# 0x002A/MuCHSALSA

Hardware: AMD Instinct MI355X
Metric: overlap-pairs/s (higher is better)
Workload: dtype int32+f64; 1 GPU; 100k synthetic Nanopore x10 kb, 500k unitig anchors, 10x coverage (BASELINE.json configs[2]); rows=5059558, reads=100000, anchors=499992, edges=981460, edgematches_rank0=25532466, orders_rank0=1029308, parallelism=one job on one GPU, edges_proven_clean_rank0=5372

## Files before the change

muchsalsa_amd/csrc/msgpu_device.h:

```cpp
#ifndef MSGPU_DEVICE_H
#define MSGPU_DEVICE_H

#include <hip/hip_runtime.h>
#include <stdint.h>

#include "msgpu.h"
#include "msgpu_internal.h"

namespace msgpu {

__device__ __forceinline__ IRow load_irow(const IRow *p) {
  const uint4 *q = reinterpret_cast<const uint4 *>(p);
  uint4        a = q[0], b = q[1];
  IRow         r;
  r.n_lo  = static_cast<int>(a.x);
  r.n_hi  = static_cast<int>(a.y);
  r.i_lo  = static_cast<int>(a.z);
  r.i_hi  = static_cast<int>(a.w);
  r.score = b.x;
  r.line  = b.y;
  r.other = b.z;
  r.pf    = b.w;
  return r;
}
__device__ __forceinline__ void store_irow(IRow *p, const IRow &r) {
  uint4 *q = reinterpret_cast<uint4 *>(p);
  q[0]     = make_uint4(static_cast<uint32_t>(r.n_lo), static_cast<uint32_t>(r.n_hi), static_cast<uint32_t>(r.i_lo),
                        static_cast<uint32_t>(r.i_hi));
  q[1]     = make_uint4(r.score, r.line, r.other, r.pf);
}

__device__ __forceinline__ IRow make_irow(const msgpu_row &row, uint32_t other, uint32_t rank) {
  IRow out;
  out.n_lo  = row.n_lo;
  out.n_hi  = row.n_hi;
  out.i_lo  = row.i_lo;
  out.i_hi  = row.i_hi;
  out.score = row.score;
  out.line  = row.line;
  out.other = other;
  out.pf    = ((row.flags & MSGPU_ROW_DIR) ? PF_DIR : 0u) | ((row.flags & MSGPU_ROW_PRIMARY) ? PF_PRIM : 0u) |
           (rank & PF_POS_MASK);
  return out;
}

__device__ __forceinline__ int rl_i32(int v, int lane) { return __builtin_amdgcn_readlane(v, lane); }
__device__ __forceinline__ uint32_t rl_u32(uint32_t v, int lane) {
  return static_cast<uint32_t>(__builtin_amdgcn_readlane(static_cast<int>(v), lane));
}
__device__ __forceinline__ uint64_t rl_u64(uint64_t v, int lane) {
  uint32_t lo = rl_u32(static_cast<uint32_t>(v), lane), hi = rl_u32(static_cast<uint32_t>(v >> 32), lane);
  return (static_cast<uint64_t>(hi) << 32) | lo;
}
__device__ __forceinline__ double rl_f64(double v, int lane) {
  return __longlong_as_double(static_cast<long long>(rl_u64(static_cast<uint64_t>(__double_as_longlong(v)), lane)));
}

__device__ __forceinline__ void publish_to_host(const HostPublish &p, int lane, uint64_t v) {
  if (!p.seq) return;
  if (lane < SC_COUNT) p.host[lane] = v;
  __threadfence_system();
  if (lane == 0) __hip_atomic_store(&p.host[SC_COUNT], p.seq, __ATOMIC_RELEASE, __HIP_MEMORY_SCOPE_SYSTEM);
}

__device__ __forceinline__ double std_max(double a, double b) { return (a < b) ? b : a; }
__device__ __forceinline__ double std_min(double a, double b) { return (b < a) ? b : a; }

__device__ __forceinline__ uint32_t wave_incl_scan(uint32_t v) {
  v += static_cast<uint32_t>(__builtin_amdgcn_update_dpp(0, static_cast<int>(v), 0x111, 0xf, 0xf, false));
  v += static_cast<uint32_t>(__builtin_amdgcn_update_dpp(0, static_cast<int>(v), 0x112, 0xf, 0xf, false));
  v += static_cast<uint32_t>(__builtin_amdgcn_update_dpp(0, static_cast<int>(v), 0x114, 0xf, 0xf, false));
  v += static_cast<uint32_t>(__builtin_amdgcn_update_dpp(0, static_cast<int>(v), 0x118, 0xf, 0xf, false));
  v += static_cast<uint32_t>(__builtin_amdgcn_update_dpp(0, static_cast<int>(v), 0x142, 0xa, 0xf, false));
  v += static_cast<uint32_t>(__builtin_amdgcn_update_dpp(0, static_cast<int>(v), 0x143, 0xc, 0xf, false));
  return v;
}

__device__ __forceinline__ uint64_t wave_incl_scan64(uint32_t v) {
  uint64_t inc = v;
  const int lane = threadIdx.x & 63;
#pragma unroll
  for (int d = 1; d < 64; d <<= 1) {
    const uint64_t t = __shfl_up(inc, d);
    if (lane >= d) inc += t;
  }
  return inc;
}
__device__ __forceinline__ uint32_t wave_sum(uint32_t v) {
  return static_cast<uint32_t>(__builtin_amdgcn_readlane(static_cast<int>(wave_incl_scan(v)), 63));
}

template <int NT> __device__ __forceinline__ uint32_t block_excl_scan(uint32_t v, uint32_t *s_wave , uint32_t *total) {
  const int      lane = threadIdx.x & 63, wave = threadIdx.x >> 6;
  const uint32_t inc  = wave_incl_scan(v);
  if (lane == 63) s_wave[wave] = inc;
  __syncthreads();
  uint32_t base = 0, tot = 0;
#pragma unroll
  for (int w = 0; w < NT / 64; ++w) {
    const uint32_t x = s_wave[w];
    base += w < wave ? x : 0u;
    tot += x;
  }
  *total = tot;
  __syncthreads();
  return base + inc - v;
}
__device__ __forceinline__ uint32_t block_excl_scan_256(uint32_t v, uint32_t *s_wave , uint32_t *total) {
  const int lane = threadIdx.x & 63, wave = threadIdx.x >> 6;
  uint32_t  inc  = v;
#pragma unroll
  for (int d = 1; d < 64; d <<= 1) {
    uint32_t t = __shfl_up(inc, d);
    if (lane >= d) inc += t;
  }
  if (lane == 63) s_wave[wave] = inc;
  __syncthreads();
  uint32_t w0 = s_wave[0], w1 = s_wave[1], w2 = s_wave[2], w3 = s_wave[3];
  uint32_t base = (wave > 0 ? w0 : 0) + (wave > 1 ? w1 : 0) + (wave > 2 ? w2 : 0);
  *total        = w0 + w1 + w2 + w3;
  __syncthreads();
  return base + inc - v;
}

__device__ __forceinline__ void note_first_row(int lane, unsigned long long key, uint32_t r, const msgpu_row *rows,
                                               int32_t *read_len, uint32_t *read_first) {
  for (int d = 32; d > 0; d >>= 1) {
    const unsigned long long o =
        (static_cast<unsigned long long>(static_cast<uint32_t>(__shfl_xor(static_cast<int>(key >> 32), d))) << 32) |
        static_cast<uint32_t>(__shfl_xor(static_cast<int>(key), d));
    key = o < key ? o : key;
  }
  if (lane == 0) {
    read_first[r] = static_cast<uint32_t>(key >> 32);
    read_len[r]   = rows[static_cast<uint32_t>(key)].read_len;
  }
}

__device__ __forceinline__ bool key_less(int alo, int ahi, uint32_t aan, int blo, int bhi, uint32_t ban) {
  return alo < blo || (alo == blo && (ahi < bhi || (ahi == bhi && aan < ban)));
}

}

#endif
```

muchsalsa_amd/csrc/msgpu_kernels.hip:

```cpp
#include <hip/hip_runtime.h>
#include <stdint.h>
#include <stdlib.h>

#include <type_traits>
#include <utility>

#include "msgpu.h"
#include "msgpu_internal.h"
#include "msgpu_device.h"

namespace msgpu {


constexpr int SCAN_ITEMS = 8;
uint32_t      scan_blocks(uint64_t n);

template <class T> __global__ __launch_bounds__(256) void k_scan_reduce(const uint32_t *in, uint64_t n, T *block_sums) {
  __shared__ T s[4];
  uint64_t     base = static_cast<uint64_t>(blockIdx.x) * 256 * SCAN_ITEMS;
  T            sum  = 0;
  for (int i = 0; i < SCAN_ITEMS; ++i) {
    uint64_t idx = base + static_cast<uint64_t>(i) * 256 + threadIdx.x;
    if (idx < n) sum += in[idx];
  }
// ... 1290 lines not shown
}
void launch_emit_edges(hipStream_t st, const EmitArgs &a, bool reduce) {
  if (reduce && a.n_chunks)
    hipLaunchKernelGGL(k_cand_reduce, dim3(a.n_chunks), dim3(1024), 0, st, a.n_edge, a.n_cand, a.cand_off, a.edge_scr_start, a.V,
                       const_cast<unsigned long long *>(a.chunk_sums), const_cast<uint32_t *>(a.hist));
  hipLaunchKernelGGL(k_emit_edges, dim3(a.n_chunks ? a.n_chunks : 1), dim3(1024), 0, st, a);
}


__device__ __forceinline__ void chunk_add(unsigned long long *chunk_sums, uint64_t e, bool clean, uint32_t n_orders, uint32_t n_ids, bool banded = false) {
  static_assert(COMPACT_CHUNK < (1u << 16), "two 16-bit edge counts in the low half of a chunk sum");
  unsigned long long *c = chunk_sums + 2 * (e / COMPACT_CHUNK);
  __hip_atomic_fetch_add(c, (clean ? 1ull : 0ull) | (banded ? 1ull << 16 : 0ull) | (static_cast<unsigned long long>(n_orders) << 32), __ATOMIC_RELAXED, __HIP_MEMORY_SCOPE_AGENT);
  __hip_atomic_fetch_add(c + 1, static_cast<unsigned long long>(n_ids), __ATOMIC_RELAXED, __HIP_MEMORY_SCOPE_AGENT);
}
__device__ __forceinline__ void band_fallback_add(unsigned long long *chunk_sums, uint64_t n_edges) {
  __hip_atomic_fetch_add(chunk_sums + 2 * (n_edges / COMPACT_CHUNK + 1), 1ull, __ATOMIC_RELAXED, __HIP_MEMORY_SCOPE_AGENT);
}

struct PathRec {
  uint64_t mask;
  uint64_t score;
  uint32_t primary;
  uint32_t pad;
};

struct __attribute__((aligned(16))) ChainElem {
  double clo1, chi1;
  double clo2, chi2;
  int    rlo1, rhi1, rlo2, rhi2;
};

struct NanoMasks {
  unsigned long long pos, neg, ovl, abort_;
};
template <bool WF, int SORTED >
__device__ __forceinline__ NanoMasks nano_check(double k_clo, double k_chi, double l_clo, double l_chi, int k_rlo,
                                                int k_rhi, int l_rlo, int l_rhi, double &d) {
  typedef unsigned long long M;
  const bool lt_lo_b = k_clo < l_clo;
  const M    lt_lo = __ballot(lt_lo_b), lt_hi = __ballot(k_chi < l_chi);
  const M    gt_lo = __ballot(k_clo > l_clo), gt_hi = __ballot(k_chi > l_chi);
  NanoMasks  f;
  const double x = k_chi - l_clo;
  const double y = l_chi - k_clo;
  double       t = lt_lo_b ? x : y;
  if (WF) {
    f.ovl = __ballot(t >= 0.0);
    d     = fabs(t) + 1;
  } else {
    f.ovl = __ballot(k_clo <= l_chi) & __ballot(l_clo <= k_chi);
    t     = __builtin_amdgcn_inverse_ballot_w64(f.ovl) ? t : -t;
    d = t + 1;
  }
  if (WF) {
    f.pos = lt_lo & lt_hi;
    f.neg = gt_lo & gt_hi;
  } else {
    f.pos = lt_lo & (lt_hi | ~f.ovl);
    f.neg = (f.ovl & gt_lo & gt_hi) | ~(f.ovl | lt_lo);
  }
  if (SORTED == 1) {
    const M rovl = __ballot(l_rlo <= k_rhi);
    const M u2   = __ballot(k_rlo < l_rlo) & __ballot(k_rhi < l_rhi);
    f.abort_     = rovl & (f.neg | (f.pos & ~u2));
  } else if (SORTED == 2) {
    const M rovl = __ballot(k_rlo <= l_rhi);
    const M um2  = __ballot(k_rlo > l_rlo) & __ballot(k_rhi > l_rhi);
    f.abort_     = rovl & (f.pos | (f.neg & ~um2));
  } else {
    const M rovl = __ballot(k_rlo <= l_rhi) & __ballot(l_rlo <= k_rhi);
    const M u2   = __ballot(k_rlo < l_rlo) & __ballot(k_rhi < l_rhi);
    const M um2  = __ballot(k_rlo > l_rlo) & __ballot(k_rhi > l_rhi);
    f.abort_     = rovl & ((f.neg & ~um2) | (f.pos & ~u2));
  }
  return f;
}

__device__ __forceinline__ int paths_of_direction(unsigned long long act, bool direction, int lane, double pop,
                                                  uint64_t pm, bool em_prim, uint32_t j1, uint32_t q2, uint32_t n1,
                                                  uint32_t n2, double alt_frac, PathRec *paths) {
  if (act == 0) return 0;
  const bool mine = (act >> lane) & 1ull;
  double best = mine ? pop : -1.0;
#pragma unroll
  for (int d = 32; d > 0; d >>= 1) best = __builtin_fmax(best, __shfl_xor(best, d));
  double maxv;
  int    maxi;
  if (best > 0.0) {
    maxv = best;
    maxi = __builtin_ctzll(__ballot(mine && pop == best));
  } else {
    maxv = 0.0;
    maxi = __builtin_ctzll(act);
  }
  maxi = __builtin_amdgcn_readfirstlane(maxi);
  const unsigned long long prim_lanes = __ballot(mine && em_prim);
  int                      np         = 0;
  const uint64_t           m          = rl_u64(pm, maxi);
  bool                     hp         = (m & prim_lanes) != 0;
  hp |= __popcll(m) > 2;
  if (lane == 0) {
    paths[0].mask    = m;
    paths[0].score   = static_cast<uint64_t>(maxv);
    paths[0].primary = hp;
  }
  np = 1;
  const double       thr  = maxv * alt_frac;
  uint64_t           used = m;
  unsigned long long cand = __ballot(mine && pop > thr);
  while (true) {
    cand &= __ballot((pm & used) == 0);
    if (!cand) break;
    const int      p  = __builtin_ctzll(cand);
    const uint64_t mp = rl_u64(pm, p);
    const double   sp = rl_f64(pop, p);
    if (lane == 0) {
      paths[np].mask    = mp;
      paths[np].score   = static_cast<uint64_t>(sp);
      paths[np].primary = (mp & prim_lanes) != 0;
    }
    ++np;
    used |= mp;
    cand &= ~(1ull << p);
  }
  if (np == 1 && hp) {
    const int first = __builtin_ctzll(m), last = 63 - __builtin_clzll(m);
    const uint32_t qe = direction ? q2 : (n2 - 1 - q2);
    const uint32_t jf = rl_u32(j1, first), jl = rl_u32(j1, last), qf = rl_u32(qe, first), ql = rl_u32(qe, last);
    bool           demote;
    if ((jf != 0 && qf != 0) || (jl != n1 - 1 && ql != n2 - 1)) {
      demote = true;
    } else {
      const bool     on   = (m >> lane) & 1ull;
      const uint64_t below = m & ((1ull << lane) - 1);
      const int      prev  = below ? 63 - __builtin_clzll(below) : lane;
      const uint32_t pj = __shfl(j1, prev), pq = __shfl(qe, prev);
      const bool     firstt = below == 0;
      const uint32_t i_t    = firstt ? 0u : pj + 1u;
      const uint32_t jj_t   = firstt ? 0u : pq + 1u;
      const bool     viol   = on && qe < jj_t;
      const unsigned long long vmask = __ballot(viol);
      const int      fv   = vmask ? __builtin_ctzll(vmask) : 64;
      const bool     i1   = j1 > i_t;
      const bool     i2   = lane < fv ? (qe > jj_t) : (lane == fv ? (n2 > jj_t) : false);
      demote              = __ballot(on && i1 && i2) != 0;
    }
    if (demote && lane == 0) paths[0].primary = 0;
  }
  return np;
}

__device__ __forceinline__ ChainElem lds_elem(uint32_t addr) {
  typedef uint32_t u32x4 __attribute__((ext_vector_type(4)));
  typedef __attribute__((address_space(3))) const u32x4 lds_u4;
  lds_u4     *q = reinterpret_cast<lds_u4 *>(static_cast<uintptr_t>(addr));
  const u32x4 a = q[0], b = q[1], c = q[2];
  ChainElem   e;
  e.clo1 = __hiloint2double(static_cast<int>(a.y), static_cast<int>(a.x));
  e.chi1 = __hiloint2double(static_cast<int>(a.w), static_cast<int>(a.z));
  e.clo2 = __hiloint2double(static_cast<int>(b.y), static_cast<int>(b.x));
  e.chi2 = __hiloint2double(static_cast<int>(b.w), static_cast<int>(b.z));
  e.rlo1 = static_cast<int>(c.x);
  e.rhi1 = static_cast<int>(c.y);
  e.rlo2 = static_cast<int>(c.z);
  e.rhi2 = static_cast<int>(c.w);
  return e;
}
constexpr uint32_t CHAIN_LDS_EL = 0, CHAIN_LDS_CM = sizeof(ChainElem) * 64, CHAIN_LDS_BYTES = CHAIN_LDS_CM + 34 * 8;
// ... 188 lines not shown
        if (__builtin_amdgcn_inverse_ballot_w64(need_div)) passd = fabs(val) * 100 / fmax(d1, d2) <= a.ratio_pct;
        ok |= __ballot(passd);
      }
      bits = ok;
    }
    {
      typedef __attribute__((address_space(3))) unsigned long long lds_u64;
      *reinterpret_cast<lds_u64 *>(static_cast<uintptr_t>(cm_addr + (step & 1) * 8u)) = bits;
    }
  };
  auto sweep = [&](auto wft, auto dirt, auto s2t) __attribute__((always_inline)) {
    pair_t ka = load_pairs(0);
    for (int p0 = 0; p0 < P; p0 += 128) {
      const pair_t kb = load_pairs(p0 + 64);
      sweep_step(p0 >> 6, ka, wft, dirt, s2t);
      if (p0 + 64 >= P) break;
      ka = load_pairs(p0 + 128);
      sweep_step((p0 >> 6) + 1, kb, wft, dirt, s2t);
      cm_addr += 16;
    }
  };
  typedef std::integral_constant<int, 0> I0;
  typedef std::integral_constant<int, 1> I1;
  typedef std::integral_constant<int, 2> I2;
  if (wf) {
    if (m_minus == 0) sweep(std::true_type{}, I0{}, I0{});
    else if (m_plus == 0) sweep(std::true_type{}, I1{}, I0{});
    else sweep(std::true_type{}, I2{}, I0{});
  } else {
    if (m_minus == 0) sweep(std::false_type{}, I0{}, I0{});
    else if (m_plus == 0) sweep(std::false_type{}, I1{}, I0{});
    else sweep(std::false_type{}, I2{}, I0{});
  }
  __builtin_amdgcn_fence(__ATOMIC_RELEASE, "wavefront");
  __builtin_amdgcn_wave_barrier();
  int ln = lane;
  asm volatile("" : "+v"(ln));
  uint64_t mycm = 0;
  if (clean) {
    mycm = act ? (1ull << ln) - 1ull : 0ull;
  } else if (act && ln > 0 && P != 0) {
    constexpr int  B  = MSGPU_CHAIN_BAND;
    const bool     tri = !band || ln <= B;
    const int      pr = tri ? ln * (ln - 1) / 2 : B * (B - 1) / 2 + (ln - B) * B, w = pr >> 6, b = pr & 63;
    const int      wd = tri ? ln : B;
    const uint64_t lo = cm[w] >> b, hi = (cm[w + 1] << 1) << (63 - b);
    mycm              = ((lo | hi) & ((1ull << wd) - 1ull)) << (ln - wd);
  }

  pop = em_score;
  pm  = 1ull << ln;
  {
    uint32_t pred = static_cast<uint32_t>(ln);
    uint32_t rev = __builtin_bitreverse32(static_cast<uint32_t>(mycm));
    const int n1 = static_cast<int>(n) - 1, nlo = n1 < 32 ? n1 : 32;
    auto dp_step = [&](int k) __attribute__((always_inline)) {
      const double       k_pop = rl_f64(pop, k);
      const double       cand  = k_pop + em_score;
      unsigned long long comp, saved;
      asm volatile("v_add_co_u32 %0, %1, %0, %0" : "+v"(rev), "=s"(comp));
      const unsigned long long upd = comp & __ballot(cand > pop);
      asm volatile("s_and_saveexec_b64 %[sv], %[m]\n\t"
                   "v_mov_b64 %[pop], %[cand]\n\t"
                   "v_mov_b32 %[pred], %[k]\n\t"
                   "s_mov_b64 exec, %[sv]"
                   : [pop] "+v"(pop), [pred] "+v"(pred), [sv] "=&s"(saved)
                   : [m] "s"(upd), [cand] "v"(cand), [k] "s"(k)
                   : "scc");
    };
    for (int k = 0; k < nlo; ++k) dp_step(k);
    rev = __builtin_bitreverse32(static_cast<uint32_t>(mycm >> 32));
    for (int k = 32; k < n1; ++k) dp_step(k);
    uint32_t ptr = pred;
    for (uint32_t span = 1; span < n; span <<= 1) {
      const uint32_t lo = __shfl(static_cast<uint32_t>(pm), static_cast<int>(ptr));
      const uint32_t hi = __shfl(static_cast<uint32_t>(pm >> 32), static_cast<int>(ptr));
      const uint32_t p2 = __shfl(ptr, static_cast<int>(ptr));
      pm |= (static_cast<uint64_t>(hi) << 32) | lo;
      ptr = p2;
    }
  }
  if (!band) break;
  {
    double pmax = pop;
#pragma unroll
    for (int d = 1; d < 64; d <<= 1) {
      const double up = __shfl_up(pmax, d);
      if (ln >= d) pmax = __builtin_fmax(pmax, up);
    }
    const double out = __shfl(pmax, ln > MSGPU_CHAIN_BAND ? ln - MSGPU_CHAIN_BAND - 1 : 0);
    const bool   rej = ln > MSGPU_CHAIN_BAND && ln < static_cast<int>(n) && !(out + em_score < pop);
    if (__ballot(rej) == 0) break;
  }
  band = false;
  if (lane == 0) band_fallback_add(a.chunk_sums, a.n_edges);
  __builtin_amdgcn_fence(__ATOMIC_RELEASE, "wavefront");
  __builtin_amdgcn_wave_barrier();
  }

  PathRec  *pmn = reinterpret_cast<PathRec *>(s_chain_lds + CHAIN_LDS_EL), *ppl = pmn + 64;
  const int n_m = paths_of_direction(m_minus, false, lane, pop, pm, em_prim, j1, q2, n1, n2, a.alt_frac, pmn);
  const int n_p = paths_of_direction(m_plus, true, lane, pop, pm, em_prim, j1, q2, n1, n2, a.alt_frac, ppl);
  __builtin_amdgcn_fence(__ATOMIC_RELEASE, "wavefront");
  __builtin_amdgcn_wave_barrier();

  bool     k_m = false, k_p = false;
  uint32_t prim_m = 0, prim_p = 0, len_m = 0, len_p = 0;
  if (lane < n_m) {
    prim_m = pmn[lane].primary;
    len_m  = static_cast<uint32_t>(__popcll(pmn[lane].mask));
    k_m    = true;
  }
  if (lane < n_p) {
    prim_p = ppl[lane].primary;
    len_p  = static_cast<uint32_t>(__popcll(ppl[lane].mask));
    k_p    = true;
  }
  const bool has_primary = __ballot((k_m && prim_m) || (k_p && prim_p)) != 0;
  if (has_primary) {
    k_m = k_m && prim_m;
    k_p = k_p && prim_p;
  }
  const bool has_multi = __ballot((k_m && len_m > 1) || (k_p && len_p > 1)) != 0;
  if (has_multi) {
    k_m = k_m && len_m > 1;
    k_p = k_p && len_p > 1;
  }
  const unsigned long long keep_m = __ballot(k_m), keep_p = __ballot(k_p);
  const int                combined = __popcll(keep_m) + __popcll(keep_p);
  bool                     shadow;
  if (combined > 1) {
    shadow = true;
  } else {
    uint32_t pr = keep_m ? rl_u32(prim_m, __builtin_ctzll(keep_m)) : rl_u32(prim_p, __builtin_ctzll(keep_p));
    shadow      = !pr;
  }

  uint32_t n_orders = 0, n_ids = 0;
  for (int pass = 0; pass < 2; ++pass) {
    unsigned long long keep = pass == 0 ? keep_m : keep_p;
    const PathRec     *pv   = pass == 0 ? pmn : ppl;
    const bool         dir  = pass == 1;
    while (keep) {
      const int pi = __builtin_ctzll(keep);
      keep &= keep - 1;
      const uint64_t mask = pv[pi].mask;
      const int      f = __builtin_ctzll(mask), l = 63 - __builtin_clzll(mask);
      const double   L1 = rl_f64(clo1, f), R1 = rl_f64(ovr1, l);
      double         L2 = rl_f64(clo2, f), R2 = rl_f64(ovr2, l);
      if (!dir) {
        L2 = rl_f64(ovr2, f);
        R2 = rl_f64(clo2, l);
      }
      bool     have = false;
      uint32_t fl   = 0;
      double   lo = 0, ro = 0;
      if (L1 <= L2 && R1 <= R2) {
        have = true;
        fl   = MSGPU_ORD_START_V1 | MSGPU_ORD_CONTAINED;
        lo   = L2 - L1;
        ro   = R2 - R1;
      } else if (L1 >= L2 && R1 >= R2) {
        have = true;
        fl   = MSGPU_ORD_CONTAINED;
        lo   = L1 - L2;
        ro   = R1 - R2;
      } else if (L1 > L2 && R1 < R2) {
        have = true;
        fl   = MSGPU_ORD_START_V1;
        lo   = L1 - L2;
        ro   = R2 - R1;
      } else if (L1 < L2 && R1 > R2) {
// ... 16 lines not shown
        o.right_offset = ro;
        o.score        = pv[pi].score;
        o.ids_off      = n_ids;
        o.ids_cnt      = cnt;
        o.start        = (fl & MSGPU_ORD_START_V1) ? v1 : v2;
        o.end          = (fl & MSGPU_ORD_START_V1) ? v2 : v1;
        o.base         = v1;
        o.pad[0]       = 0;
        o.pad[1]       = 0;
        a.order_scr[ed.em_off + n_orders] = o;
      }
      ++n_orders;
      n_ids += cnt;
    }
  }
  if (lane == 0) {
    a.edge_norders[e] = n_orders;
    a.edge_nids[e]    = n_ids;
    a.edges[e].shadow = shadow ? 1 : 0;
    chunk_add(a.chunk_sums, e, clean, n_orders, n_ids, banded);
  }
}


struct __attribute__((aligned(16))) SubPath {
  uint32_t mask, primary;
  uint64_t score;
};

__device__ __forceinline__ double shfl_f64(double v, int src) {
  const long long b  = __double_as_longlong(v);
  const uint32_t  lo = __shfl(static_cast<uint32_t>(b), src), hi = __shfl(static_cast<uint32_t>(b >> 32), src);
  return __longlong_as_double(static_cast<long long>((static_cast<unsigned long long>(hi) << 32) | lo));
}

template <int W> __device__ __forceinline__ uint32_t group_bits(unsigned long long m, int gbase) {
  return static_cast<uint32_t>(m >> gbase) & (W == 32 ? 0xffffffffu : ((1u << W) - 1u));
}

template <int W> __device__ __forceinline__ int longest_prefix(unsigned long long m) {
#pragma unroll
  for (int d = 32; d >= W; d >>= 1) m |= m >> d;
  return __popc(static_cast<uint32_t>(m) & (W == 32 ? 0xffffffffu : ((1u << W) - 1u)));
}

template <int K> __device__ __forceinline__ uint32_t row_bcast(uint32_t v) {
  static_assert(K >= 0 && K < 16, "row lane");
  return static_cast<uint32_t>(__builtin_amdgcn_mov_dpp(static_cast<int>(v), 0x150 + K, 0xf, 0xf, false));
}

template <int W, int K> __device__ __forceinline__ uint32_t group_bcast(uint32_t v) {
  static_assert(K >= 0 && K < W, "group lane");
  if constexpr (W == 16) {
    return row_bcast<K>(v);
  } else if constexpr (W == 8) {
    const int lo = __builtin_amdgcn_mov_dpp(static_cast<int>(v), 0x150 + K, 0xf, 0x3, false);
    return static_cast<uint32_t>(__builtin_amdgcn_update_dpp(lo, static_cast<int>(v), 0x150 + 8 + K, 0xf, 0xc, false));
  } else if constexpr (K < 16) {
    const int r = static_cast<int>(row_bcast<K>(v));
    return static_cast<uint32_t>(__builtin_amdgcn_update_dpp(r, r, 0x142, 0xa, 0xf, false));
  } else {
    const uint32_t r  = row_bcast<K - 16>(v);
    const uint32_t ro = static_cast<uint32_t>(__builtin_amdgcn_mov_dpp(static_cast<int>(v), 0x150 + K - 16, 0xa, 0xf, false));
    return __builtin_amdgcn_permlane16_swap(r, ro, false, false)[1];
  }
}
template <int W, int K> __device__ __forceinline__ double group_bcast_f64(double v) {
  const unsigned long long b  = __builtin_bit_cast(unsigned long long, v);
  const uint32_t           lo = group_bcast<W, K>(static_cast<uint32_t>(b));
  const uint32_t           hi = group_bcast<W, K>(static_cast<uint32_t>(b >> 32));
  return __builtin_bit_cast(double, (static_cast<unsigned long long>(hi) << 32) | lo);
}

template <typename F, int... K> __device__ __forceinline__ void unroll_while(F &&f, std::integer_sequence<int, K...>) {
  (void)(f(std::integral_constant<int, K>{}) && ...);
}

template <int W>
__device__ __forceinline__ uint32_t paths_of_direction_sub(uint32_t act, bool direction, int sl, int gbase, double pop,
                                                           uint32_t pm, bool em_prim, uint32_t j1, uint32_t q2,
                                                           uint32_t n1, uint32_t n2, double alt_frac, SubPath *paths) {
  const bool live = act != 0;
  const bool mine = (act >> sl) & 1u;
  double     best = mine ? pop : -1.0;
#pragma unroll
  for (int d = W / 2; d > 0; d >>= 1) best = __builtin_fmax(best, __shfl_xor(best, d));
  double maxv = 0.0;
  int    maxi = live ? __builtin_ctz(act) : 0;
  if (best > 0.0) {
    maxv = best;
    const uint32_t at = group_bits<W>(__ballot(mine && pop == best), gbase);
    maxi = at ? __builtin_ctz(at) : 0;
  }
  const uint32_t prim_lanes = group_bits<W>(__ballot(mine && em_prim), gbase);
  const uint32_t m          = __shfl(pm, gbase + maxi);
  const bool     hp         = ((m & prim_lanes) != 0) | (__popc(m) > 2);
  if (live && sl == 0) paths[0] = SubPath{m, hp ? 1u : 0u, static_cast<uint64_t>(maxv)};
  uint32_t np = live ? 1u : 0u;
  const double thr  = maxv * alt_frac;
  uint32_t     used = m;
  uint32_t     cand = group_bits<W>(__ballot(mine && pop > thr), gbase);
  while (true) {
    cand &= group_bits<W>(__ballot((pm & used) == 0), gbase);
    if (__ballot(cand != 0) == 0) break;
    const bool     has = cand != 0;
    const int      p   = has ? __builtin_ctz(cand) : 0;
    const uint32_t mp  = __shfl(pm, gbase + p);
    const double   sp  = shfl_f64(pop, gbase + p);
    if (has && sl == 0) paths[np] = SubPath{mp, (mp & prim_lanes) != 0 ? 1u : 0u, static_cast<uint64_t>(sp)};
    if (has) {
      ++np;
      used |= mp;
      cand &= ~(1u << p);
    }
  }
  const bool     single = live && np == 1 && hp;
  const uint32_t ms     = m ? m : 1u;
  const int      first = __builtin_ctz(ms), last = 31 - __builtin_clz(ms);
  const uint32_t qe = direction ? q2 : (n2 - 1 - q2);
  const uint32_t jf = __shfl(j1, gbase + first), jl = __shfl(j1, gbase + last);
  const uint32_t qf = __shfl(qe, gbase + first), ql = __shfl(qe, gbase + last);
  const bool     ends   = (jf != 0 && qf != 0) || (jl != n1 - 1 && ql != n2 - 1);
  const bool     on     = (m >> sl) & 1u;
  const uint32_t below  = m & ((1u << sl) - 1u);
  const int      prev   = below ? 31 - __builtin_clz(below) : sl;
  const uint32_t pj = __shfl(j1, gbase + prev), pq = __shfl(qe, gbase + prev);
  const bool     firstt = below == 0;
  const uint32_t i_t = firstt ? 0u : pj + 1u, jj_t = firstt ? 0u : pq + 1u;
  const bool     viol  = on && qe < jj_t;
  const uint32_t vmask = group_bits<W>(__ballot(viol), gbase);
  const int      fv    = vmask ? __builtin_ctz(vmask) : 64;
  const bool     i1    = j1 > i_t;
  const bool     i2    = sl < fv ? (qe > jj_t) : (sl == fv ? (n2 > jj_t) : false);
  const bool     inter = group_bits<W>(__ballot(on && i1 && i2), gbase) != 0;
  if (single && (ends || inter) && sl == 0) paths[0].primary = 0;
  return np;
}

template <int W>
__device__ __forceinline__ void chain_sub_body(const ChainArgs &a, const uint32_t *list, uint32_t n_list, uint32_t block,
                                               unsigned char (*s_wavebuf)[sizeof(ChainElem) * 64], uint32_t (*s_cm)[64],
                                               double (*s_keep)[64][4], uint32_t (*s_anchor)[64]) {
  constexpr int G = 64 / W;
  static_assert(W == 8 || W == 16 || W == 32, "group width");
  static_assert(sizeof(ChainElem) * 64 >= sizeof(SubPath) * 2 * 64, "the path lists overlay the element table");
  const int      wave = threadIdx.x >> 6, lane = threadIdx.x & 63;
  const int      g = lane / W, sl = lane % W, gbase = g * W;
  const uint32_t slot    = (block * 4 + wave) * G + g;
  const bool     valid_g = slot < n_list;
  if (__ballot(valid_g) == 0) return;
  const uint32_t   e  = valid_g ? list[slot] : list[0];
  const msgpu_edge ed = a.edges[e];
  const uint32_t   n  = (valid_g && ed.em_cnt <= static_cast<uint32_t>(W)) ? ed.em_cnt : 0u;
  const uint64_t   cp = a.edge_cand[e];
  const bool       act = sl < static_cast<int>(n);
  const uint32_t   v1 = ed.v1, v2 = ed.v2;
  const uint32_t   n1 = a.read_cnt[v1], n2 = a.read_cnt[v2];
  const int        len1 = a.read_len[v1], len2 = a.read_len[v2];
  ChainElem       *el = reinterpret_cast<ChainElem *>(s_wavebuf[wave]);
  uint32_t        *cm = s_cm[wave];

  uint32_t  j1 = 0, q2 = 0, anchor = 0;
  double    clo1 = 0, clo2 = 0, ovr1 = 0, ovr2 = 0, em_score = 0;
  bool      em_dir = false, em_prim = false;
  ChainElem x{};
  cm[lane] = 0;
  if (act) {
    j1               = a.cand_j[cp + sl];
    const uint32_t t = a.cand_t[cp + sl];
// ... 157 lines not shown
      cl &= valid;
      const double df = fabs(d1 - d2);
      const M near_ = __ballot(df <= wiggle), sum_ok = __ballot(d1 + d2 <= wiggle);
      M       ok    = cl & ((near_ & ~mixed) | (sum_ok & mixed));
      const M need_div = cl & ~(mixed | near_);
      if (need_div) {
        bool pass = false;
        if (__builtin_amdgcn_inverse_ballot_w64(need_div)) pass = df * 100 / fmax(d1, d2) <= a.ratio_pct;
        ok |= __ballot(pass);
      }
      bits = ok;
    }
    const uint32_t run = (kl.y >> 8) & 0xffu;
    if (run != 0 && in_range) {
      uint32_t *row = reinterpret_cast<uint32_t *>(cmg + (kl.y >> 16));
      __hip_atomic_fetch_or(row, __builtin_amdgcn_ubfe(static_cast<uint32_t>(bits >> lane), 0u, run) << (kl.y & 31u),
                            __ATOMIC_RELAXED, __HIP_MEMORY_SCOPE_WORKGROUP);
    }
  };
  auto sweep = [&](auto wft, auto dirt) __attribute__((always_inline)) {
    uint2 ka = load_pairs(0);
    for (int p0 = 0; p0 < Pmax; p0 += 2 * W) {
      const uint2 kb = load_pairs(p0 + W);
      sweep_step(p0, ka, wft, dirt);
      if (p0 + W >= Pmax) break;
      ka = load_pairs(p0 + 2 * W);
      sweep_step(p0 + W, kb, wft, dirt);
    }
  };
  auto sweep_dir = [&](auto wft) __attribute__((always_inline)) {
    if (!one_dir) sweep(wft, std::integral_constant<int, 2>{});
    else if (KD_one == ~0ull) sweep(wft, std::integral_constant<int, 0>{});
    else if (KD_one == 0) sweep(wft, std::integral_constant<int, 1>{});
    else sweep(wft, std::integral_constant<int, 3>{});
  };
  if (wf) sweep_dir(std::true_type{});
  else sweep_dir(std::false_type{});
  __builtin_amdgcn_fence(__ATOMIC_RELEASE, "wavefront");
  __builtin_amdgcn_wave_barrier();
  const uint32_t mycm = clean ? (act ? (1u << sl) - 1u : 0u) : cm[lane];

  const int nmax = longest_prefix<W>(__ballot(act));
  double    pop  = em_score;
  uint32_t  pm   = 1u << sl;
  {
    uint32_t pred = static_cast<uint32_t>(sl);
    uint32_t rev  = __builtin_bitreverse32(mycm);
    auto     dp_step = [&](double cand, int k) __attribute__((always_inline)) {
      unsigned long long comp, saved;
      asm volatile("v_add_co_u32 %0, %1, %0, %0" : "+v"(rev), "=s"(comp));
      const unsigned long long upd = comp & __ballot(cand > pop);
      asm volatile("s_and_saveexec_b64 %[sv], %[m]\n\t"
                   "v_mov_b64 %[pop], %[cand]\n\t"
                   "v_mov_b32 %[pred], %[k]\n\t"
                   "s_mov_b64 exec, %[sv]"
                   : [pop] "+v"(pop), [pred] "+v"(pred), [sv] "=&s"(saved)
                   : [m] "s"(upd), [cand] "v"(cand), [k] "s"(k)
                   : "scc");
    };
    unroll_while(
        [&](auto kc) __attribute__((always_inline)) {
          constexpr int k = decltype(kc)::value;
          if (k + 1 >= nmax) return false;
          dp_step(group_bcast_f64<W, k>(pop) + em_score, k);
          return true;
        },
        std::make_integer_sequence<int, W - 1>{});
    uint32_t ptr = pred;
    for (int span = 1; span < nmax; span <<= 1) {
      if constexpr (W == 32) {
        const uint32_t o  = __shfl(pm, gbase + static_cast<int>(ptr));
        const uint32_t p2 = __shfl(ptr, gbase + static_cast<int>(ptr));
        pm |= o;
        ptr = p2;
      } else {
        const uint32_t o = __shfl(pm | (ptr << 16), gbase + static_cast<int>(ptr));
        pm |= o & 0xffffu;
        ptr = o >> 16;
      }
    }
  }

  SubPath *pmn = reinterpret_cast<SubPath *>(s_wavebuf[wave]) + gbase, *ppl = pmn + 64;
  const uint32_t n_m = paths_of_direction_sub<W>(m_minus, false, sl, gbase, pop, pm, em_prim, j1, q2, n1, n2, a.alt_frac, pmn);
  const uint32_t n_p = paths_of_direction_sub<W>(m_plus, true, sl, gbase, pop, pm, em_prim, j1, q2, n1, n2, a.alt_frac, ppl);
  __builtin_amdgcn_fence(__ATOMIC_RELEASE, "wavefront");
  __builtin_amdgcn_wave_barrier();

  bool     k_m = false, k_p = false;
  uint32_t prim_m = 0, prim_p = 0, len_m = 0, len_p = 0;
  if (sl < static_cast<int>(n_m)) {
    prim_m = pmn[sl].primary;
    len_m  = static_cast<uint32_t>(__popc(pmn[sl].mask));
    k_m    = true;
  }
  if (sl < static_cast<int>(n_p)) {
    prim_p = ppl[sl].primary;
    len_p  = static_cast<uint32_t>(__popc(ppl[sl].mask));
    k_p    = true;
  }
  const bool has_primary = group_bits<W>(__ballot((k_m && prim_m) || (k_p && prim_p)), gbase) != 0;
  if (has_primary) {
    k_m = k_m && prim_m;
    k_p = k_p && prim_p;
  }
  const bool has_multi = group_bits<W>(__ballot((k_m && len_m > 1) || (k_p && len_p > 1)), gbase) != 0;
  if (has_multi) {
    k_m = k_m && len_m > 1;
    k_p = k_p && len_p > 1;
  }
  const uint32_t keep_m = group_bits<W>(__ballot(k_m), gbase), keep_p = group_bits<W>(__ballot(k_p), gbase);
  const int      combined = __popc(keep_m) + __popc(keep_p);
  bool           shadow   = true;
  if (combined == 1) shadow = !(keep_m ? pmn[__builtin_ctz(keep_m)].primary : ppl[__builtin_ctz(keep_p)].primary);

  uint32_t n_orders = 0, n_ids = 0;
  for (int pass = 0; pass < 2; ++pass) {
    uint32_t       keep = pass == 0 ? keep_m : keep_p;
    const SubPath *pv   = pass == 0 ? pmn : ppl;
    const bool     dir  = pass == 1;
    while (__ballot(keep != 0)) {
      const bool has = keep != 0;
      const int  pi  = has ? __builtin_ctz(keep) : 0;
      keep &= keep - 1u;
      const SubPath  rec  = pv[pi];
      const uint32_t mask = (has && rec.mask) ? rec.mask : 1u;
      const int      f = __builtin_ctz(mask), l = 31 - __builtin_clz(mask);
      const double  *kf = s_keep[wave][gbase + f], *kl = s_keep[wave][gbase + l];
      const double   L1 = kf[0], R1 = kl[2];
      const double   L2 = dir ? kf[1] : kf[3], R2 = dir ? kl[3] : kl[1];
      bool     have = false;
      uint32_t fl   = 0;
      double   lo = 0, ro = 0;
      if (L1 <= L2 && R1 <= R2) {
        have = true;
        fl   = MSGPU_ORD_START_V1 | MSGPU_ORD_CONTAINED;
        lo   = L2 - L1;
        ro   = R2 - R1;
      } else if (L1 >= L2 && R1 >= R2) {
        have = true;
        fl   = MSGPU_ORD_CONTAINED;
        lo   = L1 - L2;
        ro   = R1 - R2;
      } else if (L1 > L2 && R1 < R2) {
        have = true;
        fl   = MSGPU_ORD_START_V1;
        lo   = L1 - L2;
        ro   = R2 - R1;
      } else if (L1 < L2 && R1 > R2) {
        have = true;
        fl   = 0;
        lo   = L2 - L1;
        ro   = R1 - R2;
      }
      const bool emit = has && have;
      if (emit) {
        const uint32_t cnt = static_cast<uint32_t>(__popc(mask));
        if ((mask >> sl) & 1u) a.ids_scr[ed.em_off + n_ids + static_cast<uint32_t>(__popc(mask & ((1u << sl) - 1u)))] = s_anchor[wave][lane];
        if (sl == 0) {
          msgpu_order o;
          o.edge_idx     = e;
          o.flags        = fl | (dir ? MSGPU_ORD_DIR : 0u) | (rec.primary ? MSGPU_ORD_PRIMARY : 0u);
          o.left_offset  = lo;
          o.right_offset = ro;
          o.score        = rec.score;
          o.ids_off      = n_ids;
          o.ids_cnt      = cnt;
          o.start        = (fl & MSGPU_ORD_START_V1) ? v1 : v2;
          o.end          = (fl & MSGPU_ORD_START_V1) ? v2 : v1;
          o.base         = v1;
          o.pad[0]       = 0;
          o.pad[1]       = 0;
          a.order_scr[ed.em_off + n_orders] = o;
        }
        ++n_orders;
        n_ids += cnt;
      }
    }
  }
  if (n && sl == 0) {
    a.edge_norders[e] = n_orders;
    a.edge_nids[e]    = n_ids;
    a.edges[e].shadow = shadow ? 1 : 0;
    chunk_add(a.chunk_sums, e, clean, n_orders, n_ids);
  }
}

template <int W>
__global__ __launch_bounds__(256) __attribute__((amdgpu_waves_per_eu(W == 32 ? 7 : 6, W == 32 ? 7 : 6))) void k_chain_sub(ChainArgs a, const uint32_t *list, uint32_t n_list) {
  __shared__ __attribute__((aligned(16))) unsigned char s_wavebuf[4][sizeof(ChainElem) * 64];
  __shared__ uint32_t                                  s_cm[4][64];
  __shared__ __attribute__((aligned(16))) double       s_keep[4][64][4];
  __shared__ uint32_t                                  s_anchor[4][64];
  chain_sub_body<W>(a, list, n_list, blockIdx.x, s_wavebuf, s_cm, s_keep, s_anchor);
}
#ifndef MSGPU_SUB_WAVES
#define MSGPU_SUB_WAVES 7
#endif
__global__ __launch_bounds__(256) __attribute__((amdgpu_waves_per_eu(MSGPU_SUB_WAVES, MSGPU_SUB_WAVES))) void k_chain_sub_all(ChainArgs a, ChainSubLists l) {
  __shared__ __attribute__((aligned(16))) unsigned char s_wavebuf[4][sizeof(ChainElem) * 64];
  __shared__ uint32_t                                  s_cm[4][64];
  __shared__ __attribute__((aligned(16))) double       s_keep[4][64][4];
  __shared__ uint32_t                                  s_anchor[4][64];
  uint32_t b = blockIdx.x;
  if (b < l.nb32) {
    chain_sub_body<32>(a, l.list32, l.n32, b, s_wavebuf, s_cm, s_keep, s_anchor);
  } else if ((b -= l.nb32) < l.nb16) {
    chain_sub_body<16>(a, l.list16, l.n16, b, s_wavebuf, s_cm, s_keep, s_anchor);
// ... 968 lines not shown
```

Before: 428.5 million overlap-pairs/s.

## Use DPP/permlane f64 max reductions and merge per-direction path loops

Replaces shfl-based f64 max reductions and the prefix-max scan with DPP row operations and permlane16/32 swaps, avoiding LDS-backed bpermute traffic. In the sub-wave path builder, the two direction calls are folded into a loop that runs only once when no group has both directions active. The order-emission loop also walks the minus and plus keep masks in a single combined loop, so groups with uneven work no longer serialise two separate divergent loops. This adds control-flow complexity and relies on gfx950-specific permlane swap builtins; the masking of the merged loops must exactly preserve the original semantics.

```diff
diff --git a/muchsalsa_amd/csrc/msgpu_device.h b/muchsalsa_amd/csrc/msgpu_device.h
--- a/muchsalsa_amd/csrc/msgpu_device.h
+++ b/muchsalsa_amd/csrc/msgpu_device.h
@@ -90,6 +90,52 @@
   return static_cast<uint32_t>(__builtin_amdgcn_readlane(static_cast<int>(wave_incl_scan(v)), 63));
 }
 
+template <int CTRL, int ROW_MASK = 0xf, bool PERMUTES = false> __device__ __forceinline__ double dpp_max_step(double v) {
+  const unsigned long long b  = __builtin_bit_cast(unsigned long long, v);
+  const int                lo = static_cast<int>(static_cast<uint32_t>(b)), hi = static_cast<int>(static_cast<uint32_t>(b >> 32));
+  uint32_t                 ml, mh;
+  if constexpr (PERMUTES) {
+    static_assert(ROW_MASK == 0xf, "every row takes part in a permutation");
+    ml = static_cast<uint32_t>(__builtin_amdgcn_mov_dpp(lo, CTRL, 0xf, 0xf, false));
+    mh = static_cast<uint32_t>(__builtin_amdgcn_mov_dpp(hi, CTRL, 0xf, 0xf, false));
+  } else {
+    ml = static_cast<uint32_t>(__builtin_amdgcn_update_dpp(lo, lo, CTRL, ROW_MASK, 0xf, false));
+    mh = static_cast<uint32_t>(__builtin_amdgcn_update_dpp(hi, hi, CTRL, ROW_MASK, 0xf, false));
+  }
+  return __builtin_fmax(v, __builtin_bit_cast(double, (static_cast<unsigned long long>(mh) << 32) | ml));
+}
+template <int W> __device__ __forceinline__ double group_max_f64(double v) {
+  static_assert(W == 8 || W == 16 || W == 32 || W == 64, "group width");
+  v = dpp_max_step<0xb1, 0xf, true>(v);
+  v = dpp_max_step<0x4e, 0xf, true>(v);
+  v = dpp_max_step<0x141, 0xf, true>(v);
+  if constexpr (W >= 16) v = dpp_max_step<0x140, 0xf, true>(v);
+  if constexpr (W >= 32) {
+    const unsigned long long b  = __builtin_bit_cast(unsigned long long, v);
+    const auto               lo = __builtin_amdgcn_permlane16_swap(static_cast<uint32_t>(b), static_cast<uint32_t>(b), false, false);
+    const auto               hi = __builtin_amdgcn_permlane16_swap(static_cast<uint32_t>(b >> 32), static_cast<uint32_t>(b >> 32), false, false);
+    v = __builtin_fmax(__builtin_bit_cast(double, (static_cast<unsigned long long>(hi[0]) << 32) | lo[0]),
+                       __builtin_bit_cast(double, (static_cast<unsigned long long>(hi[1]) << 32) | lo[1]));
+  }
+  if constexpr (W == 64) {
+    const unsigned long long b  = __builtin_bit_cast(unsigned long long, v);
+    const auto               lo = __builtin_amdgcn_permlane32_swap(static_cast<uint32_t>(b), static_cast<uint32_t>(b), false, false);
+    const auto               hi = __builtin_amdgcn_permlane32_swap(static_cast<uint32_t>(b >> 32), static_cast<uint32_t>(b >> 32), false, false);
+    v = __builtin_fmax(__builtin_bit_cast(double, (static_cast<unsigned long long>(hi[0]) << 32) | lo[0]),
+                       __builtin_bit_cast(double, (static_cast<unsigned long long>(hi[1]) << 32) | lo[1]));
+  }
+  return v;
+}
+__device__ __forceinline__ double wave_prefix_max_f64(double v) {
+  v = dpp_max_step<0x111>(v);
+  v = dpp_max_step<0x112>(v);
+  v = dpp_max_step<0x114>(v);
+  v = dpp_max_step<0x118>(v);
+  v = dpp_max_step<0x142, 0xa>(v);
+  v = dpp_max_step<0x143, 0xc>(v);
+  return v;
+}
+
 template <int NT> __device__ __forceinline__ uint32_t block_excl_scan(uint32_t v, uint32_t *s_wave , uint32_t *total) {
   const int      lane = threadIdx.x & 63, wave = threadIdx.x >> 6;
   const uint32_t inc  = wave_incl_scan(v);
diff --git a/muchsalsa_amd/csrc/msgpu_kernels.hip b/muchsalsa_amd/csrc/msgpu_kernels.hip
--- a/muchsalsa_amd/csrc/msgpu_kernels.hip
+++ b/muchsalsa_amd/csrc/msgpu_kernels.hip
@@ -1396,9 +1396,7 @@
                                                   uint32_t n2, double alt_frac, PathRec *paths) {
   if (act == 0) return 0;
   const bool mine = (act >> lane) & 1ull;
-  double best = mine ? pop : -1.0;
-#pragma unroll
-  for (int d = 32; d > 0; d >>= 1) best = __builtin_fmax(best, __shfl_xor(best, d));
+  const double best = group_max_f64<64>(mine ? pop : -1.0);
   double maxv;
   int    maxi;
   if (best > 0.0) {
@@ -1753,12 +1751,7 @@
   }
   if (!band) break;
   {
-    double pmax = pop;
-#pragma unroll
-    for (int d = 1; d < 64; d <<= 1) {
-      const double up = __shfl_up(pmax, d);
-      if (ln >= d) pmax = __builtin_fmax(pmax, up);
-    }
+    const double pmax = wave_prefix_max_f64(pop);
     const double out = __shfl(pmax, ln > MSGPU_CHAIN_BAND ? ln - MSGPU_CHAIN_BAND - 1 : 0);
     const bool   rej = ln > MSGPU_CHAIN_BAND && ln < static_cast<int>(n) && !(out + em_score < pop);
     if (__ballot(rej) == 0) break;
@@ -1941,9 +1934,7 @@
                                                            uint32_t n1, uint32_t n2, double alt_frac, SubPath *paths) {
   const bool live = act != 0;
   const bool mine = (act >> sl) & 1u;
-  double     best = mine ? pop : -1.0;
-#pragma unroll
-  for (int d = W / 2; d > 0; d >>= 1) best = __builtin_fmax(best, __shfl_xor(best, d));
+  const double best = group_max_f64<W>(mine ? pop : -1.0);
   double maxv = 0.0;
   int    maxi = live ? __builtin_ctz(act) : 0;
   if (best > 0.0) {
@@ -2267,8 +2258,15 @@
   }
 
   SubPath *pmn = reinterpret_cast<SubPath *>(s_wavebuf[wave]) + gbase, *ppl = pmn + 64;
-  const uint32_t n_m = paths_of_direction_sub<W>(m_minus, false, sl, gbase, pop, pm, em_prim, j1, q2, n1, n2, a.alt_frac, pmn);
-  const uint32_t n_p = paths_of_direction_sub<W>(m_plus, true, sl, gbase, pop, pm, em_prim, j1, q2, n1, n2, a.alt_frac, ppl);
+  uint32_t n_m = 0, n_p = 0;
+#pragma clang loop unroll(disable)
+  for (int trip = 0; trip < 2; ++trip) {
+    const bool     dir  = trip != 0 || m_minus == 0;
+    const uint32_t actd = trip == 0 ? (m_minus ? m_minus : m_plus) : (m_minus ? m_plus : 0u);
+    const uint32_t np   = paths_of_direction_sub<W>(actd, dir, sl, gbase, pop, pm, em_prim, j1, q2, n1, n2, a.alt_frac, dir ? ppl : pmn);
+    if (actd) (dir ? n_p : n_m) = np;
+    if (__ballot(m_minus != 0 && m_plus != 0) == 0) break;
+  }
   __builtin_amdgcn_fence(__ATOMIC_RELEASE, "wavefront");
   __builtin_amdgcn_wave_barrier();
 
@@ -2300,15 +2298,16 @@
   if (combined == 1) shadow = !(keep_m ? pmn[__builtin_ctz(keep_m)].primary : ppl[__builtin_ctz(keep_p)].primary);
 
   uint32_t n_orders = 0, n_ids = 0;
-  for (int pass = 0; pass < 2; ++pass) {
-    uint32_t       keep = pass == 0 ? keep_m : keep_p;
-    const SubPath *pv   = pass == 0 ? pmn : ppl;
-    const bool     dir  = pass == 1;
-    while (__ballot(keep != 0)) {
-      const bool has = keep != 0;
-      const int  pi  = has ? __builtin_ctz(keep) : 0;
-      keep &= keep - 1u;
-      const SubPath  rec  = pv[pi];
+  {
+    uint32_t km = keep_m, kp = keep_p;
+    while (__ballot((km | kp) != 0)) {
+      const bool     dir  = km == 0;
+      const uint32_t keep = dir ? kp : km;
+      const bool     has  = keep != 0;
+      const int      pi   = has ? __builtin_ctz(keep) : 0;
+      km &= km - 1u;
+      kp = dir ? (keep & (keep - 1u)) : kp;
+      const SubPath  rec  = (dir ? ppl : pmn)[pi];
       const uint32_t mask = (has && rec.mask) ? rec.mask : 1u;
       const int      f = __builtin_ctz(mask), l = 31 - __builtin_clz(mask);
       const double  *kf = s_keep[wave][gbase + f], *kl = s_keep[wave][gbase + l];
```

Result: faster. 438.8 million overlap-pairs/s (median of 6 runs) (+2.4%).
